# JuliaGaussianProcesses/AbstractGPs.jl

Hardware: AMD Instinct MI355X
Metric: logpdf+posterior throughput (points/sec, fp64) at N=65536; % MFMA roofline (higher is better)
Workload: dtype f64; 1 GPU; C4: GP(SqExponentialKernel()) on 65536 3-D points, sigma2=0.01, fp64, one (logpdf, posterior-fit) pair per step; n=65536, d=3, parallelism=1 GPU

## Files before the change

abstractgps.jl_amd/csrc/bulk_plan.hpp:

```cpp
#pragma once
#include <algorithm>
#include <cstddef>
#include <vector>

namespace gpmi {

static inline double lower_count(long M, long N, long row0, long col0) {
    const long a = row0 - col0 + 1;
    const long i1 = std::min(std::max(1 - a, 0L), M);
    const long i2 = std::max(i1, std::min(std::max(N - a, 0L), M));
    const double mid = (double)(i2 - i1) * (double)a + 0.5 * (double)(i1 + i2 - 1) * (double)(i2 - i1);
    return mid + (double)(M - i2) * (double)N;
}

static inline bool strassen_shape_rule(long min_rows, long M, long N, long K) {
    return min_rows > 0 && std::min(M, N) >= std::max(256L, min_rows) && M % 256 == 0 && N % 256 == 0 && K % 32 == 0;
}
static inline long strassen_split_rule(long min_rows, long m, long K) {
    const long h = (m / 2) / 256 * 256;
    return strassen_shape_rule(min_rows, h, h, K) ? h : 0;
}
static inline size_t strassen_ws_rule(long ldpad, long M, long N, long K) { return (size_t)5 * (size_t)(M / 2 + N / 2) * (size_t)(K / 2 + ldpad); }
static inline long plan_tiles(long M, long N, int lower) {
    const long tm = (M + 127) / 128, tn = (N + 127) / 128;
// ... 38 lines not shown
    size_t ws_elems = 0;
    std::vector<PlanLaunch> ungrouped;
    size_t nprobs() const { return list[0].size() + list[1].size() + list[2].size() + list[3].size(); }
};

namespace plan_detail {
struct Builder {
    BulkPlan& p;
    long min_rows, ldpad;
    std::vector<PlanProb> classical;

    void rect(long c_off, long a_off, long b_off, long M, long N) {
        if (M <= 0 || N <= 0) return;
        PlanProb e{};
        e.c_off = c_off; e.a_off = a_off; e.b_off = b_off;
        e.M = M; e.N = N; e.K = p.K;
        e.block = -1;
        classical.push_back(e);
        p.ungrouped.push_back(PlanLaunch{0, M, N, p.K, 1, 0});
    }
    void product(int launch, int product, int block, long c_off, long c2off, int s1, int s2, int a_src, long a_off, int b_src, long b_off, long mh, long nh, long kh) {
        PlanProb e{};
        e.c_off = c_off; e.a_off = a_off; e.b_off = b_off;
        e.a_src = a_src; e.b_src = b_src;
        e.M = mh; e.N = nh; e.K = kh;
        e.beta0 = 1; e.c2off = c2off; e.s1 = s1; e.s2 = s2;
        e.block = block; e.product = product;
        p.list[launch].push_back(e);
    }
    void strassen(long c_off, long a_off, long b_off, long M, long N) {
        const long K = p.K;
        if (!strassen_shape_rule(min_rows, M, N, K)) return rect(c_off, a_off, b_off, M, N);
        const long mh = M / 2, nh = N / 2, kh = K / 2, lds = p.lds, ldp = p.ldp;
        const long pa = mh * lds, pb = nh * lds;
        const int bi = (int)p.blocks.size();
        const long sa = (long)p.ws_elems, sb = sa + 5 * pa;
        p.blocks.push_back(PlanBlock{c_off, a_off, b_off, M, N, K, sa, 5 * (pa + pb)});
        p.ws_elems += (size_t)(5 * (pa + pb));
        p.sums.push_back(PlanSums{a_off, mh, kh, 0, sa, pa});
        p.sums.push_back(PlanSums{b_off, nh, kh, 1, sb, pb});
        const long dn = nh, dm = mh * p.ldc;
        product(0, 1, bi, c_off, dm + dn, 1, 1, 1, sa, 1, sb, mh, nh, kh);
        product(1, 2, bi, c_off + dm, dn, 1, -1, 1, sa + pa, 0, b_off, mh, nh, kh);
        product(1, 5, bi, c_off + dn, -dn, 1, -1, 1, sa + 2 * pa, 0, b_off + nh * ldp + kh, mh, nh, kh);
        product(2, 3, bi, c_off + dn, dm, 1, 1, 0, a_off, 1, sb + pb, mh, nh, kh);
        product(2, 4, bi, c_off, dm, 1, 1, 0, a_off + mh * ldp + kh, 1, sb + 2 * pb, mh, nh, kh);
        product(3, 6, bi, c_off + dm + dn, 0, 1, 0, 1, sa + 3 * pa, 1, sb + 3 * pb, mh, nh, kh);
        product(3, 7, bi, c_off, 0, 1, 0, 1, sa + 4 * pa, 1, sb + 4 * pb, mh, nh, kh);
        p.ungrouped.push_back(PlanLaunch{1, mh, kh, 0, 1, 0});
        p.ungrouped.push_back(PlanLaunch{1, nh, kh, 0, 1, 0});
        p.ungrouped.push_back(PlanLaunch{0, mh, nh, kh, 1, 0});
        for (int i = 0; i < 3; ++i) p.ungrouped.push_back(PlanLaunch{0, mh, nh, kh, 2, 0});
    }
    void syrk(long roff, long mrows, long m) {
        const long K = p.K, ldc = p.ldc, ldp = p.ldp;
        const long h = strassen_split_rule(min_rows, m, K);
        if (h == 0) {
            PlanProb e{};
            e.c_off = roff * ldc + roff; e.a_off = roff * ldp; e.b_off = roff * ldp;
            e.M = mrows; e.N = m; e.K = K;
            e.lower = 1; e.roff = roff;
            e.block = -1;
            classical.push_back(e);
            p.ungrouped.push_back(PlanLaunch{0, mrows, m, K, 1, 1});
            return;
        }
        const long b = m - h, bs = b / 256 * 256;
        syrk(roff, h, h);
        strassen((roff + h) * ldc + roff, (roff + h) * ldp, roff * ldp, bs, h);
        if (b > bs) rect((roff + h + bs) * ldc + roff, (roff + h + bs) * ldp, roff * ldp, b - bs, h);
        syrk(roff + h, b, b);
        if (mrows > m) rect((roff + m) * ldc + roff, (roff + m) * ldp, roff * ldp, mrows - m, m);
    }
};
}

static inline BulkPlan bulk_plan_build(long mrows, long m, long K, long row0, long ldc, long ldp, long min_rows, long ldpad) {
    BulkPlan p;
    p.mrows = mrows; p.m = m; p.K = K; p.row0 = row0; p.ldc = ldc; p.ldp = ldp;
    p.lds = K / 2 + ldpad;
    plan_detail::Builder bd{p, min_rows, ldpad, {}};
    bd.syrk(0, mrows, m);
    double work[4];
    for (int l = 0; l < 4; ++l) {
        work[l] = 0;
        for (auto& e : p.list[l]) work[l] += (double)plan_tiles(e.M, e.N, e.lower) * (double)e.K;
    }
    std::stable_sort(bd.classical.begin(), bd.classical.end(), [](const PlanProb& a, const PlanProb& b) {
        return plan_tiles(a.M, a.N, a.lower) * a.K > plan_tiles(b.M, b.N, b.lower) * b.K;
    });
    for (auto& e : bd.classical) {
        int l = 0;
        for (int i = 1; i < 4; ++i)
            if (work[i] < work[l]) l = i;
        work[l] += (double)plan_tiles(e.M, e.N, e.lower) * (double)e.K;
        p.list[l].push_back(e);
    }
    for (int l = 0; l < 4; ++l) {
        std::stable_sort(p.list[l].begin(), p.list[l].end(), [](const PlanProb& a, const PlanProb& b) {
            if (a.K != b.K) return a.K > b.K;
            return plan_tiles(a.M, a.N, a.lower) > plan_tiles(b.M, b.N, b.lower);
        });
        long t = 0;
        for (auto& e : p.list[l]) {
            e.tile0 = t;
            e.ntiles = plan_tiles(e.M, e.N, e.lower);
            t += e.ntiles;
            const double elems = e.lower ? lower_count(e.M, e.N, row0 + e.roff, row0 + e.roff) : (double)e.M * (double)e.N;
            p.flops[l] += 2.0 * (double)e.K * elems;
            p.bytes[l] += 16.0 * elems * (e.c2off ? 2 : 1) + 8.0 * (double)e.K * (double)(e.M + e.N);
        }
        p.ntiles[l] = t;
    }
    return p;
}

struct GrpProb {
    double* C;
    const double* A;
    const double* B;
    long ldc, lda, ldb;
    long row0, col0;
    long c2off;
    int M, N, K;
    int lower, tn, beta0, s1, s2;
    int tile0;
    int pad_[5];
};
static_assert(sizeof(GrpProb) == 128, "one table entry is 128 bytes");

static inline GrpProb plan_entry(const BulkPlan& p, const PlanProb& e, double* C, const double* P, const double* ws) {
    GrpProb q{};
    q.C = C + e.c_off;
    q.A = (e.a_src ? ws : P) + e.a_off;
    q.B = (e.b_src ? ws : P) + e.b_off;
    q.ldc = p.ldc;
    q.lda = e.a_src ? p.lds : p.ldp;
    q.ldb = e.b_src ? p.lds : p.ldp;
    q.row0 = q.col0 = e.lower ? p.row0 + e.roff : 0;
    q.c2off = e.c2off;
    q.M = (int)e.M; q.N = (int)e.N; q.K = (int)e.K;
    q.lower = e.lower;
    q.tn = (int)((e.N + 127) / 128);
    q.beta0 = e.beta0; q.s1 = e.s1; q.s2 = e.s2;
    q.tile0 = (int)e.tile0;
    return q;
}

}
```

abstractgps.jl_amd/csrc/engine.hpp:

```cpp
#pragma once
#include <hip/hip_runtime.h>
#include <stdint.h>

#include <array>
#include <atomic>
#include <memory>
#include <mutex>
#include <set>
#include <string>
#include <unordered_map>
#include <vector>

#include "../../include/gpmi355.h"
#include "bulk_plan.hpp"

namespace gpmi {
struct GridMap {
    int lower;
    int P, p, Q, q;
    long nb;
    long row0, col0;
    int compact;
    int tn, dt;
    int tm;
// ... 11 lines not shown
struct KSum {
    enum { MAXT = 8, MAXFT = 4, MAXF = 16, MAXTH = 64, MAXD = 16 };
    int nterms, nth;
    int t0[MAXT + 1];
    int tv[MAXT];
    int kind[MAXF];
    int ns[MAXF];
    int so[MAXF];
    int po[MAXF];
    double th[MAXTH];
};
static_assert(sizeof(KSum) < 1024, "the composite kernel descriptor travels as a kernel argument");
}

int32_t set_hip_err(hipError_t e, const char* what, int line);
int32_t set_arg_err(int i, const char* msg);
int32_t set_err_text(int32_t status, const std::string& msg);
#define HIPCHK(expr)                                                   \
    do {                                                               \
        hipError_t e_ = (expr);                                        \
        if (e_ != hipSuccess) return set_hip_err(e_, #expr, __LINE__); \
    } while (0)
#define RC(expr)                \
    do {                        \
        int32_t rc_ = (expr);   \
        if (rc_ != 0) return rc_; \
    } while (0)

static inline long round_up(long v, long m) { return (v + m - 1) / m * m; }
static const double LOG2PI = 1.8378770664093454835606594728112;

template <class F> static inline auto by_dtype(int dtype, F&& f) { return dtype == 0 ? f(double()) : f(float()); }
static inline void put(void* out, int dtype, size_t i, double v) {
    if (dtype == 0) ((double*)out)[i] = v;
    else ((float*)out)[i] = (float)v;
}

struct FreeBlock {
    void* p;
    size_t bytes;
};

struct gp_ctx {
    int device = 0;
    hipStream_t sm = nullptr;
    hipStream_t sp = nullptr;
    void* pin = nullptr;
    size_t pin_bytes = 0;
    hipStream_t sq = nullptr;
    bool own_sm = false;
    std::mutex mu;
    long nb = -1;
    long nb_small = 4096, nb_large = 2048;
    int lookahead = 1;
    long lookahead_min_n = 24576;
    int time_kernels = 0;
    int sched = 0;
    long trsv_nb = 256;
    long leaf_group = 128;
    int deterministic = 0;
    int leaf_v2 = 1;
    int leaf_xr = 0;
    int upd128 = 1;
    long updk_max_k = 512;
    long updk_tall_k = 256;
    long updk_tall_m = 8192;
    int updk_rt = 0;
    int leaf_cols = 128;
    int gemm_streamk = 1;
    int num_cus = 256;
    long sk_max_tiles = 4096;
    long sk_min_k = 0;
    int sk_scope = 0;
    long gemm_pad_lds = 0;
    long gemm_pad_f32 = 0;
    int gemm_pipe = 1;
    long dib_nb = 2048;
    bool gemm_pad_set = false;
    bool gemm_pad_user = false;
    long vfe_ks = 2048;
    int vfe_overlap = 1;
    int vfe_sk = 0;
    int vfe_dual = 0;
    long vfe_inv_nb = 512;
    long strassen_min_rows = 8192;
    long strassen_min_rows_large = 4096;
    bool strassen_min_rows_set = false;
    long strassen_v = 8192;
    int strassen_group = 1;
    long strassen_group_min_rows = 8192;
    void* plan_pin = nullptr;
    size_t plan_pin_bytes = 0;
    hipEvent_t plan_ev = nullptr;
    bool grp_pad_set = false;
    int xcd_swizzle = 0;
    long xcd_min_tiles = 256;
    long ldpad = 32;
    long dense_stage_mb = 64;
    gp_timings tm{};
    std::vector<FreeBlock> pool;
    std::unordered_map<void*, size_t> blk;
    size_t pool_bytes = 0;
    size_t pool_cap = (size_t)96 << 30;
    int alloc_poison = 0;
    int64_t batch_grad_problems = 0;
    int64_t batch_pgrad_problems = 0;
    int64_t batch_gradx_problems = 0;
    int64_t batch_joint_problems = 0;
    long vfe_chunk = 0;
    std::vector<hipEvent_t> ev_pool;
    size_t ev_used = 0;
    struct GemmRec {
        hipEvent_t a, b;
        double flops, bytes;
        long M, N, K;
        long nprob, ntiles;
        int stream;
    };
    std::vector<GemmRec> gemm_recs;
    hipEvent_t ev_phase[4] = {nullptr, nullptr, nullptr, nullptr};
    int* info_dev = nullptr;
    int* ticket_dev = nullptr;
    void* w_ws = nullptr;
    size_t w_ws_bytes = 0;
    double* scal_dev = nullptr;
    long scal_cap = 0;
    std::atomic<int> refs{1};
    bool dead = false;
    struct gp_multi* multi = nullptr;
};

struct SkScope {
    gp_ctx* c;
    explicit SkScope(gp_ctx* c_) : c(c_) { ++c->sk_scope; }
    ~SkScope() { --c->sk_scope; }
};


extern std::mutex g_reg_mu;
extern std::set<void*> g_live;
void reg_add(void* p);
bool reg_take(void* p);
bool reg_has(void* p);
// ... 175 lines not shown
```

abstractgps.jl_amd/csrc/gpmi355.hip:

```cpp
#include "kernels.hpp"

#include <algorithm>
#include <atomic>
#include <cmath>
#include <cstdio>
#include <cstdlib>
#include <cstring>
#include <mutex>
#include <set>
#include <memory>
#include <string>
#include <thread>
#include <type_traits>
#include <unordered_map>
#include <vector>

using namespace gpmi;

static thread_local std::string g_err;
int32_t set_err_text(int32_t status, const std::string& msg) {
    g_err = msg;
    return status;
}
int32_t set_hip_err(hipError_t e, const char* what, int line) {
// ... 318 lines not shown
        g.c2stride = c2s;
        g.s1 = s1;
        g.s2 = s2;
        g.nbatch = nb;
        g.cstride = cs;
        g.astride = as;
        g.bstride = bs;
        return launch_gemm<double>(c, s, c1, ldc, a, la, b, lb, mh, nh, kh, g);
    };
    const long dn = nh, dm = mh * ldc;
    RC(prod(1, C, 0, dm + dn, 0, 1, 1, SA, lds, 0, SB, lds, 0));
    RC(prod(2, C + dm, dn - dm, dn, -2 * dn, 1, -1, SA + pa, lds, pa, B, ldb, nh * ldb + kh));
    RC(prod(2, C + dn, -dn, dm, 0, 1, 1, A, lda, mh * lda + kh, SB + pb, lds, pb));
    RC(prod(2, C + dm + dn, -(dm + dn), 0, 0, 1, 0, SA + 3 * pa, lds, pa, SB + 3 * pb, lds, pb));
    return 0;
}

static int32_t syrk_lower_split(gp_ctx* c, hipStream_t s, const StrassenWs& ws, double* C, long ldc, const double* P, long ldp, long mrows, long m, long K,
                                long row0) {
    const long h = ws.p ? strassen_split(c, m, K) : 0;
    if (h == 0) return launch_gemm<double>(c, s, C, ldc, P, ldp, P, ldp, mrows, m, K, plain_map(1, row0, row0));
    const long b = m - h, bs = b / 256 * 256;
    RC(syrk_lower_split(c, s, ws, C, ldc, P, ldp, h, h, K, row0));
    RC(gemm_nt_strassen(c, s, ws, C + h * ldc, ldc, P + h * ldp, ldp, P, ldp, bs, h, K));
    if (b > bs) RC(launch_gemm<double>(c, s, C + (h + bs) * ldc, ldc, P + (h + bs) * ldp, ldp, P, ldp, b - bs, h, K, plain_map(0, 0, 0)));
    RC(syrk_lower_split(c, s, ws, C + h * ldc + h, ldc, P + h * ldp, ldp, b, b, K, row0 + h));
    if (mrows > m) RC(launch_gemm<double>(c, s, C + m * ldc, ldc, P + m * ldp, ldp, P, ldp, mrows - m, m, K, plain_map(0, 0, 0)));
    return 0;
}
static size_t syrk_split_ws_elems(const gp_ctx* c, long m, long K) {
    return strassen_split(c, m, K) ? strassen_ws_elems(c, m / 2 + 256, m / 2 + 256, K) : 0;
}

static bool group_applies(const gp_ctx* c, long m, long K, long ldp, const double* P) {
    return c->strassen_group && !c->xcd_swizzle && m >= c->strassen_group_min_rows && strassen_split(c, m, K) != 0 && ldp % 2 == 0 && ((uintptr_t)P & 15) == 0;
}
struct GroupedUpdate {
    BulkPlan plan;
    const double* P = nullptr;
    size_t tab0[4] = {0, 0, 0, 0};
};
struct PlanTables {
    std::vector<GroupedUpdate> upd;
    std::vector<GrpProb> host;
    size_t ws_elems = 0;
    GrpProb* dev = nullptr;
    void add(const gp_ctx* c, long mrows, long m, long K, long row0, long ldc, const double* P, long ldp) {
        GroupedUpdate u;
        u.plan = bulk_plan_build(mrows, m, K, row0, ldc, ldp, c->strassen_v, c->ldpad);
        u.P = P;
        ws_elems = std::max(ws_elems, u.plan.ws_elems);
        upd.push_back(std::move(u));
    }
    int32_t upload(gp_ctx* c, hipStream_t s, DevBufs& bufs, const std::vector<double*>& Cs, const double* ws) {
        for (size_t i = 0; i < upd.size(); ++i)
            for (int l = 0; l < 4; ++l) {
                upd[i].tab0[l] = host.size();
                for (const PlanProb& e : upd[i].plan.list[l]) host.push_back(plan_entry(upd[i].plan, e, Cs[i], upd[i].P, ws));
            }
        if (host.empty()) return 0;
        const size_t bytes = host.size() * sizeof(GrpProb);
        void* p = nullptr;
        RC(bufs.get(bytes, &p));
        dev = (GrpProb*)p;
        if (!c->plan_ev) HIPCHK(hipEventCreateWithFlags(&c->plan_ev, hipEventDisableTiming));
        HIPCHK(hipEventSynchronize(c->plan_ev));
        if (c->plan_pin_bytes < bytes) {
            if (c->plan_pin) (void)hipHostFree(c->plan_pin);
            c->plan_pin = nullptr;
            c->plan_pin_bytes = 0;
            HIPCHK(hipHostMalloc(&c->plan_pin, bytes + bytes / 4 + 4096, hipHostMallocDefault));
            c->plan_pin_bytes = bytes + bytes / 4 + 4096;
        }
        memcpy(c->plan_pin, host.data(), bytes);
        HIPCHK(hipMemcpyAsync(dev, c->plan_pin, bytes, hipMemcpyHostToDevice, s));
        HIPCHK(hipEventRecord(c->plan_ev, s));
        return 0;
    }
};

static int32_t launch_gemm_grp(gp_ctx* c, hipStream_t s, const GrpProb* tab, long nprob, long ntiles, double flops, double bytes, long K) {
    if (nprob <= 0 || ntiles <= 0) return 0;
    gp_ctx::GemmRec rec{};
    const bool timed = c->time_kernels != 0;
    if (timed) {
        RC(ctx_event(c, &rec.a, true));
        RC(ctx_event(c, &rec.b, true));
        rec.flops = flops;
        rec.bytes = bytes;
        rec.M = 0; rec.N = 0; rec.K = K;
        rec.nprob = nprob; rec.ntiles = ntiles;
        rec.stream = (s == c->sp);
        HIPCHK(hipEventRecord(rec.a, s));
    }
    const long pad = c->gemm_pad_user ? c->gemm_pad_lds : 0;
    if (pad > 0 && !c->grp_pad_set) {
        HIPCHK(hipFuncSetAttribute((const void*)gemm_nt_grp_kernel<double, 0>, hipFuncAttributeMaxDynamicSharedMemorySize, 32768));
        HIPCHK(hipFuncSetAttribute((const void*)gemm_nt_grp_kernel<double, 1>, hipFuncAttributeMaxDynamicSharedMemorySize, 32768));
        c->grp_pad_set = true;
    }
    if (c->gemm_pipe) hipLaunchKernelGGL((gemm_nt_grp_kernel<double, 1>), dim3((unsigned)ntiles), dim3(256), (size_t)pad, s, tab, (int)nprob);
    else hipLaunchKernelGGL((gemm_nt_grp_kernel<double, 0>), dim3((unsigned)ntiles), dim3(256), (size_t)pad, s, tab, (int)nprob);
    HIPCHK(hipGetLastError());
    if (timed) {
        HIPCHK(hipEventRecord(rec.b, s));
        c->gemm_recs.push_back(rec);
// ... 292 lines not shown
static int32_t trsm_back_cached(gp_ctx* c, hipStream_t s, T* X, long ldx, long M, long Mvalid, const T* A, long ld, long np, const DibCache& cache,
                                DevBufs& bufs, BackWs& ws) {
    if (M <= 0 || Mvalid <= 0) return 0;
    if (!cache.w || cache.nbi < 128 || c->dib_nb < 128) return trsv<T>(c, s, A, ld, np, X, ldx, (int)Mvalid, false);
    const long nbi = cache.nbi, ldw = cache.ldw;
    if (!ws.bt) {
        const size_t wb = sizeof(T) * (size_t)(np + 128) * ldw;
        void* S_probe = nullptr;
        if (bufs.get(wb, &ws.bt) != 0 || bufs.scratch(sizeof(T) * (size_t)(M + 128) * ldw, &S_probe) != 0) {
            ws.bt = nullptr;
            return trsv<T>(c, s, A, ld, np, X, ldx, (int)Mvalid, false);
        }
        HIPCHK(hipMemsetAsync(ws.bt, 0, wb, s));
    }
    void* S_v = nullptr;
    RC(bufs.scratch(sizeof(T) * (size_t)(M + 128) * ldw, &S_v));
    T* Bt = (T*)ws.bt;
    T* S = (T*)S_v;
    const T* W = (const T*)cache.w;
    std::vector<std::pair<long, long>> blocks;
    dib_ranges(0, np, nbi, blocks);
    for (long bi = (long)blocks.size() - 1; bi >= 0; --bi) {
        const long j0 = blocks[bi].first, n = blocks[bi].second;
        hipLaunchKernelGGL(transpose_rect_kernel<T>, dim3((unsigned)((n + 31) / 32), (unsigned)((n + 31) / 32)), dim3(256), 0, s, W + j0 * ldw, ldw, Bt, ldw, n, n, 1);
        HIPCHK(hipGetLastError());
        GridMap g = plain_map(0, 0, 0);
        g.beta0 = 1;
        RC(launch_gemm<T>(c, s, S, ldw, X + j0, ldx, Bt, ldw, M, n, n, g));
        HIPCHK(hipMemcpy2DAsync(X + j0, sizeof(T) * ldx, S, sizeof(T) * ldw, sizeof(T) * n, M, hipMemcpyDeviceToDevice, s));
        if (j0 > 0) {
            hipLaunchKernelGGL(transpose_rect_kernel<T>, dim3((unsigned)((j0 + 31) / 32), (unsigned)((n + 31) / 32)), dim3(256), 0, s, A + j0 * ld, ld, Bt, ldw, n, j0, 0);
            HIPCHK(hipGetLastError());
            RC(launch_gemm<T>(c, s, X, ldx, X + j0, ldx, Bt, ldw, M, j0, n, plain_map(0, 0, 0)));
        }
    }
    return 0;
}

template <typename T>
static int32_t potrf_full_la(gp_ctx* c, T* A, long lda, long np, long mtot, int* info_dev, long n_valid, double* logdet_dev, DevBufs* bufs);

template <typename T>
static int32_t potrf_full(gp_ctx* c, T* A, long lda, long np, long mtot, int* info_dev, long n_valid,
                          double* logdet_dev, DevBufs* bufs = nullptr) {
    if (c->nb == 0) return potrf_rec<T>(c, c->sm, A, lda, 0, np, mtot, info_dev, 0, n_valid, logdet_dev);
    return potrf_full_la<T>(c, A, lda, np, mtot, info_dev, n_valid, logdet_dev, bufs);
}

template <typename T>
static int32_t potrf_full_la(gp_ctx* c, T* A, long lda, long np, long mtot, int* info_dev, long n_valid,
                             double* logdet_dev, DevBufs* bufs) {
    long nb = c->nb;
    c->strassen_v = (!c->strassen_min_rows_set && np >= c->lookahead_min_n) ? c->strassen_min_rows_large : c->strassen_min_rows;
    if (nb < 0) nb = np < c->lookahead_min_n ? c->nb_small : c->nb_large;
    if (nb <= 0 || nb >= np) return potrf_rec<T>(c, c->sm, A, lda, 0, np, mtot, info_dev, 0, n_valid, logdet_dev);
    nb = round_up(nb, 128);
    const bool la = c->lookahead != 0 && np >= c->lookahead_min_n;
    hipStream_t sM = c->sm, sP = la ? c->sp : c->sm;
    hipEvent_t ev_u1 = nullptr, ev_panel = nullptr;
    StrassenWs ws;
    PlanTables tabs;
    std::vector<long> gidx;
    if constexpr (std::is_same<T, double>::value) {
        if (bufs) {
            size_t el = 0;
            std::vector<double*> Cs;
            for (long k = 0; k < np; k += nb) {
                const long nbk = std::min(nb, np - k), k1 = k + nbk;
                if (k1 >= np) break;
                const long k2 = k1 + std::min(nb, np - k1);
                long gi = -1;
                if (k2 < np) {
                    const double* P = A + k2 * lda + k;
                    if (group_applies(c, np - k2, nbk, lda, P)) {
                        gi = (long)tabs.upd.size();
                        tabs.add(c, mtot - k2, np - k2, nbk, k2, lda, P, lda);
                        Cs.push_back(A + k2 * lda + k2);
                    } else
                        el = std::max(el, syrk_split_ws_elems(c, np - k2, nbk));
                }
                gidx.push_back(gi);
            }
            el = std::max(el, tabs.ws_elems);
            if (el) {
                void* p = nullptr;
                RC(bufs->get(sizeof(double) * el, &p));
                ws.p = (double*)p;
                ws.elems = el;
            }
            RC(tabs.upload(c, c->sm, *bufs, Cs, ws.p));
        }
    }
    if (la) {
        RC(ctx_event(c, &ev_u1, false));
        HIPCHK(hipEventRecord(ev_u1, c->sm));
        HIPCHK(hipStreamWaitEvent(sP, ev_u1, 0));
    }
    for (long k = 0; k < np; k += nb) {
        const long nbk = std::min(nb, np - k);
        RC(potrf_rec<T>(c, sP, A, lda, k, nbk, mtot, info_dev, 0, n_valid, logdet_dev));
        const long k1 = k + nbk;
        if (la) {
            RC(ctx_event(c, &ev_panel, false));
            HIPCHK(hipEventRecord(ev_panel, sP));
            HIPCHK(hipStreamWaitEvent(sM, ev_panel, 0));
        }
        if (k1 >= np) break;
        const long nb1 = std::min(nb, np - k1);
        RC(launch_gemm<T>(c, sM, A + k1 * lda + k1, lda, A + k1 * lda + k, lda, A + k1 * lda + k, lda, mtot - k1, nb1, nbk, plain_map(1, k1, k1)));
        if (la) {
            RC(ctx_event(c, &ev_u1, false));
            HIPCHK(hipEventRecord(ev_u1, sM));
            HIPCHK(hipStreamWaitEvent(sP, ev_u1, 0));
        }
        const long k2 = k1 + nb1;
        if (k2 < np) {
            if constexpr (std::is_same<T, double>::value) {
                const size_t step = (size_t)(k / nb);
                if (step < gidx.size() && gidx[step] >= 0) RC(run_grouped(c, sM, tabs, (size_t)gidx[step], ws.p));
                else RC(syrk_lower_split(c, sM, ws, A + k2 * lda + k2, lda, A + k2 * lda + k, lda, mtot - k2, np - k2, nbk, k2));
            } else
                RC(launch_gemm<T>(c, sM, A + k2 * lda + k2, lda, A + k2 * lda + k, lda, A + k2 * lda + k, lda,
                                  mtot - k2, np - k2, nbk, plain_map(1, k2, k2)));
        }
    }
    return 0;
}

template <typename T>
static int32_t trsv(gp_ctx* c, hipStream_t s, const T* L, long ldl, long np, T* R, long ldr, int nrhs, bool fwd) {
    const int NBV = (int)c->trsv_nb;
    const bool k2 = NBV <= 256;
    const size_t smem = k2 ? sizeof(T) * (256 + 64 * 65 + 16 * 64 + 4 * 256) : sizeof(T) * (NBV + 64 * 65 + 16 * 64);
    const long nblk = (np + NBV - 1) / NBV;
    T* W = nullptr;
    RC(trtri_tiles<T>(c, s, L, ldl, np, &W));
    for (long bb = 0; bb < nblk; ++bb) {
        const long b = fwd ? bb : (nblk - 1 - bb);
        const long b0 = b * NBV;
        const int nbv = (int)std::min<long>(NBV, np - b0);
        if (fwd) {
            if (k2)
                hipLaunchKernelGGL((trsv_diag2_kernel<T, true>), dim3(1), dim3(1024), smem, s, L, ldl, b0, nbv, R, ldr, nrhs, (const T*)W);
            else
                hipLaunchKernelGGL((trsv_diag_kernel<T, true>), dim3(1), dim3(1024), smem, s, L, ldl, b0, nbv, R, ldr, nrhs, (const T*)W);
            HIPCHK(hipGetLastError());
            const long lo = b0 + nbv;
            if (lo < np) {
                hipLaunchKernelGGL(trsv_upd_fwd_kernel<T>, dim3((unsigned)((np - lo + 3) / 4)), dim3(256), 0, s, L,
                                   ldl, b0, nbv, lo, np, R, ldr, nrhs);
                HIPCHK(hipGetLastError());
            }
        } else {
            if (k2)
                hipLaunchKernelGGL((trsv_diag2_kernel<T, false>), dim3(1), dim3(1024), smem, s, L, ldl, b0, nbv, R, ldr, nrhs, (const T*)W);
            else
                hipLaunchKernelGGL((trsv_diag_kernel<T, false>), dim3(1), dim3(1024), smem, s, L, ldl, b0, nbv, R, ldr, nrhs, (const T*)W);
            HIPCHK(hipGetLastError());
            if (b0 > 0) {
                hipLaunchKernelGGL(trsv_upd_bwd_kernel<T>, dim3((unsigned)((b0 + 255) / 256), c->deterministic ? 1u : (unsigned)(nbv / 64)),
                                   dim3(256), 0, s, L, ldl, b0, nbv, R, ldr, nrhs);
                HIPCHK(hipGetLastError());
// ... 1103 lines not shown
        if (hipGetDeviceProperties(&prop, device) == hipSuccess && prop.multiProcessorCount > 0) c->num_cus = prop.multiProcessorCount;
    }
    int lo = 0, hi = 0;
    (void)hipDeviceGetStreamPriorityRange(&lo, &hi);
    hipError_t e = hipStreamCreateWithPriority(&c->sp, hipStreamNonBlocking, hi);
    if (e != hipSuccess) {
        if (c->own_sm) (void)hipStreamDestroy(c->sm);
        delete c;
        return set_hip_err(e, "hipStreamCreateWithPriority", __LINE__);
    }
    reg_add(c);
    *out = c;
    if (const char* s = getenv("GPMI_PARAMS")) {
        std::string all(s);
        size_t pos = 0;
        while (pos < all.size()) {
            size_t e = all.find(',', pos);
            if (e == std::string::npos) e = all.size();
            const std::string kv = all.substr(pos, e - pos);
            const size_t q = kv.find('=');
            if (q != std::string::npos) (void)gp_ctx_set_param(c, kv.substr(0, q).c_str(), atoll(kv.c_str() + q + 1));
            pos = e + 1;
        }
    }
    return 0;
}

int32_t gp_ctx_destroy(gp_ctx* c) {
    if (!c || !reg_take(c)) return set_arg_err(1, "not a live gp_ctx");
    gp_multi* multi = nullptr;
    {
        std::lock_guard<std::mutex> l(c->mu);
        (void)hipSetDevice(c->device);
        (void)hipStreamSynchronize(c->sm);
        (void)hipStreamSynchronize(c->sp);
        c->dead = true;
        multi = c->multi;
        c->multi = nullptr;
    }
    if (multi) multi_destroy(multi);
    (void)hipSetDevice(c->device);
    ctx_unref(c);
    return 0;
}

int32_t gp_ctx_set_param(gp_ctx* c, const char* name, int64_t v) {
    Guard gd(c);
    if (!gd.ok) return set_arg_err(1, "not a live gp_ctx");
    if (!name) return set_arg_err(2, "name is NULL");
    if (c->multi && multi_set_param(c, name, v) == 0) return 0;
    if (!strcmp(name, "nb")) c->nb = v < 0 ? -1 : (v == 0 ? 0 : round_up(v, 128));
    else if (!strcmp(name, "nb_small")) c->nb_small = (v <= 0) ? 0 : round_up(v, 128);
    else if (!strcmp(name, "nb_large")) c->nb_large = (v <= 0) ? 0 : round_up(v, 128);
    else if (!strcmp(name, "lookahead")) c->lookahead = v != 0;
    else if (!strcmp(name, "lookahead_min_n")) c->lookahead_min_n = std::max<int64_t>(0, v);
    else if (!strcmp(name, "time_kernels")) c->time_kernels = v != 0;
    else if (!strcmp(name, "xcd_swizzle")) c->xcd_swizzle = v != 0;
    else if (!strcmp(name, "strassen_min_rows")) {
        c->strassen_min_rows = v <= 0 ? 0 : round_up(v, 256);
        c->strassen_min_rows_set = true;
    } else if (!strcmp(name, "strassen_min_rows_large")) c->strassen_min_rows_large = v <= 0 ? 0 : round_up(v, 256);
    else if (!strcmp(name, "strassen_group")) c->strassen_group = v != 0;
    else if (!strcmp(name, "strassen_group_min_rows")) c->strassen_group_min_rows = std::max<int64_t>(256, round_up(v, 256));
    else if (!strcmp(name, "gemm_streamk")) c->gemm_streamk = v != 0;
    else if (!strcmp(name, "sk_max_tiles")) c->sk_max_tiles = v;
    else if (!strcmp(name, "sk_min_k")) c->sk_min_k = v;
    else if (!strcmp(name, "gemm_pipe")) c->gemm_pipe = v != 0;
    else if (!strcmp(name, "kmat_rows")) g_kmat_rows = v != 0;
    else if (!strcmp(name, "dib_nb")) c->dib_nb = v <= 0 ? 0 : std::min<int64_t>(round_up(std::max<int64_t>(v, 128), 128), 8192);
    else if (!strcmp(name, "gemm_pad_f32")) c->gemm_pad_f32 = std::min<int64_t>(std::max<int64_t>(0, v), 32768);
    else if (!strcmp(name, "gemm_pad_lds")) {
        c->gemm_pad_lds = std::min<int64_t>(std::max<int64_t>(0, v), 32768);
        c->gemm_pad_user = true;
    }
    else if (!strcmp(name, "trsv_nb")) c->trsv_nb = v >= 1024 ? 1024 : (v >= 512 ? 512 : (v >= 256 ? 256 : 128));
    else if (!strcmp(name, "deterministic")) c->deterministic = v != 0;
    else if (!strcmp(name, "leaf_v2")) c->leaf_v2 = v != 0;
    else if (!strcmp(name, "leaf_xr")) c->leaf_xr = v == 64 ? 64 : (v == 128 ? 128 : 0);
    else if (!strcmp(name, "leaf_cols")) c->leaf_cols = v == 64 ? 64 : 128;
    else if (!strcmp(name, "updk_max_k")) c->updk_max_k = std::max<int64_t>(0, v);
    else if (!strcmp(name, "updk_rt")) c->updk_rt = (int)v;
    else if (!strcmp(name, "updk_tall_k")) c->updk_tall_k = std::max<int64_t>(0, v);
    else if (!strcmp(name, "updk_tall_m")) c->updk_tall_m = std::max<int64_t>(0, v);
    else if (!strcmp(name, "upd128")) c->upd128 = v != 0;
    else if (!strcmp(name, "leaf_group")) c->leaf_group = v < 128 ? 64 : (v >= 512 ? 512 : (v >= 256 ? 256 : 128));
    else if (!strcmp(name, "xcd_min_tiles")) c->xcd_min_tiles = v;
    else if (!strcmp(name, "ldpad")) c->ldpad = round_up(std::max<int64_t>(0, v), 16);
    else if (!strcmp(name, "dense_stage_mb")) c->dense_stage_mb = std::min<int64_t>(std::max<int64_t>(1, v), 256);
    else if (!strcmp(name, "vfe_ks")) c->vfe_ks = std::max<int64_t>(512, round_up(v, 512));
    else if (!strcmp(name, "vfe_sk")) c->vfe_sk = v != 0;
    else if (!strcmp(name, "vfe_dual")) c->vfe_dual = v != 0;
    else if (!strcmp(name, "vfe_inv_nb")) c->vfe_inv_nb = v <= 0 ? 0 : round_up(v, 128);
    else if (!strcmp(name, "vfe_overlap")) c->vfe_overlap = v != 0;
    else if (!strcmp(name, "vfe_chunk")) c->vfe_chunk = v <= 0 ? 0 : std::max<int64_t>(2048, round_up(v, 2048));
    else if (!strcmp(name, "pool_cap_mb")) c->pool_cap = (size_t)std::max<int64_t>(0, v) << 20;
    else if (!strcmp(name, "alloc_poison")) c->alloc_poison = v != 0;
    else if (!strcmp(name, "lookahead_depth") || !strcmp(name, "dist_nb") || !strcmp(name, "copy_kernel") || !strcmp(name, "multi_debug_sync") ||
             !strcmp(name, "multi_check") || !strcmp(name, "multi_verify") || !strcmp(name, "multi_inject_fault") || !strcmp(name, "multi_dist_predict") || !strcmp(name, "multi_window") || !strcmp(name, "multi_timeout_s") || !strcmp(name, "multi_gemm_streamk") || !strcmp(name, "multi_leaf_cols")) return c->multi ? 0 : set_arg_err(2, "multi-device parameter on a single-device ctx");
    else return set_arg_err(2, "unknown parameter");
    return 0;
}

int32_t gp_ctx_get_param(gp_ctx* c, const char* name, int64_t* out) {
    Guard gd(c);
    if (!gd.ok) return set_arg_err(1, "not a live gp_ctx");
    if (!name) return set_arg_err(2, "name is NULL");
    if (!out) return set_arg_err(3, "out is NULL");
    if (c->multi && multi_get_param(c, name, out) == 0) return 0;
    if (!strcmp(name, "batch_grad_kernel_problems")) {
        *out = c->batch_grad_problems;
        return 0;
    }
    if (!strcmp(name, "batch_pgrad_kernel_problems")) {
        *out = c->batch_pgrad_problems;
        return 0;
    }
    if (!strcmp(name, "batch_gradx_kernel_problems")) {
        *out = c->batch_gradx_problems;
        return 0;
    }
    if (!strcmp(name, "batch_joint_kernel_problems")) {
        *out = c->batch_joint_problems;
        return 0;
    }
    const struct { const char* n; int64_t v; } tab[] = {
        {"nb", c->nb}, {"nb_small", c->nb_small}, {"nb_large", c->nb_large}, {"lookahead", c->lookahead}, {"lookahead_min_n", c->lookahead_min_n}, {"time_kernels", c->time_kernels},
        {"xcd_swizzle", c->xcd_swizzle}, {"strassen_min_rows", c->strassen_min_rows}, {"strassen_min_rows_large", c->strassen_min_rows_large}, {"strassen_group", c->strassen_group}, {"strassen_group_min_rows", c->strassen_group_min_rows}, {"xcd_min_tiles", c->xcd_min_tiles}, {"gemm_streamk", c->gemm_streamk},
        {"sk_max_tiles", c->sk_max_tiles}, {"sk_min_k", c->sk_min_k}, {"gemm_pipe", c->gemm_pipe}, {"gemm_pad_f32", c->gemm_pad_f32},
        {"gemm_pad_lds", c->gemm_pad_user ? c->gemm_pad_lds : 0}, {"trsv_nb", c->trsv_nb},  {"deterministic", c->deterministic},
        {"leaf_v2", c->leaf_v2}, {"leaf_xr", c->leaf_xr}, {"leaf_cols", c->leaf_cols}, {"updk_max_k", c->updk_max_k}, {"updk_rt", c->updk_rt},
        {"updk_tall_k", c->updk_tall_k}, {"updk_tall_m", c->updk_tall_m}, {"upd128", c->upd128}, {"leaf_group", c->leaf_group},
        {"ldpad", c->ldpad}, {"dense_stage_mb", c->dense_stage_mb}, {"vfe_ks", c->vfe_ks}, {"vfe_sk", c->vfe_sk}, {"vfe_dual", c->vfe_dual}, {"vfe_inv_nb", c->vfe_inv_nb}, {"vfe_overlap", c->vfe_overlap}, {"vfe_chunk", c->vfe_chunk},
        {"kmat_rows", g_kmat_rows.load()}, {"dib_nb", c->dib_nb}, {"pool_cap_mb", (int64_t)(c->pool_cap >> 20)}, {"alloc_poison", c->alloc_poison},
        {"pool_cached_mb", (int64_t)(c->pool_bytes >> 20)}, {"pool_blocks", (int64_t)c->pool.size()}};
    for (const auto& e : tab)
        if (!strcmp(name, e.n)) {
            *out = e.v;
            return 0;
        }
    return set_arg_err(2, "unknown parameter");
}

int32_t gp_ctx_trim(gp_ctx* c) {
    Guard gd(c);
    if (!gd.ok) return set_arg_err(1, "not a live gp_ctx");
    (void)hipSetDevice(c->device);
    (void)hipStreamSynchronize(c->sm);
    (void)hipStreamSynchronize(c->sp);
    while (!c->pool.empty()) pool_drop(c, c->pool.size() - 1);
    if (c->multi) multi_trim(c);
    return 0;
}

int32_t gp_get_timings(gp_ctx* c, gp_timings* out) {
    Guard gd(c);
    if (!gd.ok) return set_arg_err(1, "not a live gp_ctx");
    if (!out) return set_arg_err(2, "out is NULL");
    *out = c->tm;
    return 0;
}

extern "C++" int32_t pack_ksum(const gp_ksum* k, int d, int argi, KSum& ks, gp_kernel& kid) {
    if (!k) return set_arg_err(argi, "kernel is NULL");
    if (k->dtype != 0 && k->dtype != 1) return set_arg_err(argi, "dtype must be 0 (f64) or 1 (f32)");
    if (k->nterms < 1 || k->nterms > KSum::MAXT) return set_arg_err(argi, "composite kernel: 1..8 terms");
    if (!k->terms) return set_arg_err(argi, "composite kernel: terms is NULL");
    if (d > KSum::MAXD) return set_arg_err(argi, "composite kernel: D must be <= 16");
    ks = KSum{};
    int nf = 0, nth = 0;
    double vsum = 0;
    const char* too_many = "composite kernel: at most 64 entries in theta";
    for (int t = 0; t < k->nterms; ++t) {
        const gp_kterm& tm = k->terms[t];
        if (!(tm.variance > 0)) return set_arg_err(argi, "composite kernel: term variance must be > 0");
        if (tm.nfactors < 1 || tm.nfactors > KSum::MAXFT) return set_arg_err(argi, "composite kernel: 1..4 factors per term");
        if (!tm.factors) return set_arg_err(argi, "composite kernel: factors is NULL");
        if (nf + tm.nfactors > KSum::MAXF) return set_arg_err(argi, "composite kernel: at most 16 factors in all");
        if (nth >= KSum::MAXTH) return set_arg_err(argi, too_many);
        ks.t0[t] = nf;
// ... 1045 lines not shown
```

include/gpmi355.h:

```cpp
#ifndef GPMI355_H
#define GPMI355_H

#include <stdint.h>

#ifdef __cplusplus
extern "C" {
#endif

#define GPMI355_ABI_VERSION 4

typedef struct gp_ctx gp_ctx;
typedef struct gp_post gp_post;
typedef struct gp_vfe gp_vfe;

typedef struct {
    int32_t kind;
    int32_t dtype;
    double variance;
    int32_t nscale;
    const double* scale;
} gp_kernel;

typedef struct {
    int32_t kind;
    int32_t nscale;
    const double* scale;
    int32_t nparam;
    const double* param;
} gp_kfactor;
typedef struct {
    double variance;
    int32_t nfactors;
    const gp_kfactor* factors;
} gp_kterm;
typedef struct {
    int32_t dtype;
    int32_t nterms;
    const gp_kterm* terms;
} gp_ksum;

typedef struct {
    const void* data;
    int64_t n;
    int32_t d;
    int32_t layout;
} gp_points;

typedef struct {
    int32_t kind;
    double s;
    const void* diag;
} gp_noise;

typedef struct {
    double assemble_ms;
    double potrf_ms;
    double solve_ms;
    double total_ms;
    double gemm_ms;
    double gemm_flops;
    int64_t gemm_launches;
    double gemm_bytes;
} gp_timings;

int32_t gp_ctx_create(gp_ctx** out, int32_t device, void* stream_or_null);
int32_t gp_ctx_create_multi(gp_ctx** out, const int32_t* devices, int32_t ndev, int32_t P, int32_t Q, int32_t nb);
int32_t gp_ctx_multi_info(gp_ctx* ctx, int32_t* P, int32_t* Q, int32_t* nb, int32_t* comm, int32_t* depth);
int32_t gp_ctx_multi_stats(gp_ctx* ctx, int64_t* fits, int64_t* retries, int64_t* solves);
int32_t gp_multi_solve_trace(int32_t P, int32_t Q, int32_t nblk, const char* path);
int32_t gp_multi_solve_trace_ex(int32_t P, int32_t Q, int32_t nblk, int32_t flags, const char* path);
int32_t gp_multi_schedule_trace(int32_t P, int32_t Q, int32_t nblk, int32_t depth, int32_t comm, const char* path);
int32_t gp_ctx_destroy(gp_ctx* ctx);
#define GPMI355_PARAM_DEFAULTS                                                                                                   \
    "nb=-1,nb_small=4096,nb_large=2048,lookahead=1,lookahead_min_n=24576,time_kernels=0,xcd_swizzle=0,xcd_min_tiles=256,gemm_streamk=1,sk_max_tiles=4096," \
    "sk_min_k=0,gemm_pipe=1,gemm_pad_f32=0,gemm_pad_lds=0,trsv_nb=256,deterministic=0,leaf_v2=1,leaf_xr=0,leaf_cols=128,"    \
    "updk_max_k=512,updk_rt=0,updk_tall_k=256,updk_tall_m=8192,upd128=1,leaf_group=128,ldpad=32,vfe_ks=2048,vfe_sk=0,"          \
    "vfe_overlap=1,vfe_dual=0,vfe_inv_nb=512,vfe_chunk=0,kmat_rows=1,dib_nb=2048,pool_cap_mb=98304,dense_stage_mb=64,alloc_poison=0,strassen_min_rows=8192,strassen_min_rows_large=4096,strassen_group=1,strassen_group_min_rows=8192"
int32_t gp_ctx_set_param(gp_ctx* ctx, const char* name, int64_t value);
int32_t gp_ctx_get_param(gp_ctx* ctx, const char* name, int64_t* value_out);
int32_t gp_ctx_trim(gp_ctx* ctx);
int32_t gp_get_timings(gp_ctx* ctx, gp_timings* out);
const char* gp_last_error(void);
int32_t gp_abi_version(void);

int32_t gp_kernelmatrix(gp_ctx* ctx, const gp_kernel* k, const gp_points* x, const gp_points* y_or_null,
                        void* out);

int32_t gp_logpdf(gp_ctx* ctx, const gp_kernel* k, const gp_points* x, const gp_noise* noise,
                  const void* mean_or_null, const void* Y, int64_t ldy, int32_t ncols, void* out);

int32_t gp_logpdf_terms(gp_ctx* ctx, const gp_kernel* k, const gp_points* x, const gp_noise* noise, const void* mean_or_null,
                        const void* Y_or_null, int64_t ldy, int32_t ncols, void* logdet_out_or_null, void* sqmahal_out_or_null);

int32_t gp_posterior_fit(gp_ctx* ctx, const gp_kernel* k, const gp_points* x, const gp_noise* noise,
                         const void* mean_or_null, const void* y, gp_post** out, void* alpha_out_or_null,
                         void* logpdf_out_or_null);

int32_t gp_posterior_predict(gp_post* post, const gp_points* xs, const void* prior_mean_xs_or_null,
                             int32_t what, void* mean_out, void* var_out, void* cov_out);
int32_t gp_posterior_predict_grad(gp_post* post, const gp_points* xs, const void* prior_mean_xs_or_null, int32_t what,
                                  void* mean_out_or_null, void* var_out_or_null, void* dmean_out_or_null, void* dvar_out_or_null);
int32_t gp_posterior_logpdf(gp_post* post, const gp_points* xs, const void* prior_mean_xs_or_null, const gp_noise* noise,
                            const void* Y, int64_t ldy, int32_t ncols, void* out);
int32_t gp_posterior_rand(gp_post* post, const gp_points* xs, const void* prior_mean_xs_or_null, const gp_noise* noise,
                          const void* xi, int32_t ncols, void* out);

int32_t gp_logpdf_grad(gp_ctx* ctx, const gp_kernel* k, const gp_points* x, const gp_noise* noise, const void* mean_or_null,
                       const void* y, void* logpdf_out, double* dvariance_out, double* dscale_out, void* dnoise_out,
                       void* dy_out, void* dx_out);

int32_t gp_kernelmatrix_sum(gp_ctx* ctx, const gp_ksum* k, const gp_points* x, const gp_points* y_or_null, void* out);
int32_t gp_logpdf_sum(gp_ctx* ctx, const gp_ksum* k, const gp_points* x, const gp_noise* noise, const void* mean_or_null,
                      const void* Y, int64_t ldy, int32_t ncols, void* out);
int32_t gp_posterior_fit_sum(gp_ctx* ctx, const gp_ksum* k, const gp_points* x, const gp_noise* noise, const void* mean_or_null,
                             const void* y, gp_post** out, void* alpha_out_or_null, void* logpdf_out_or_null);
int32_t gp_logpdf_grad_sum(gp_ctx* ctx, const gp_ksum* k, const gp_points* x, const gp_noise* noise, const void* mean_or_null,
                           const void* y, void* logpdf_out, double* dtheta_out_or_null, void* dnoise_out_or_null,
                           void* dy_out_or_null);
int32_t gp_logpdf_grad_sum_x(gp_ctx* ctx, const gp_ksum* k, const gp_points* x, const gp_noise* noise, const void* mean_or_null,
                             const void* y, void* logpdf_out, double* dtheta_out_or_null, void* dnoise_out_or_null,
                             void* dy_out_or_null, void* dx_out_or_null);
int32_t gp_logpdf_terms_sum(gp_ctx* ctx, const gp_ksum* k, const gp_points* x, const gp_noise* noise, const void* mean_or_null,
                            const void* Y_or_null, int64_t ldy, int32_t ncols, void* logdet_out_or_null, void* sqmahal_out_or_null);

#define GPMI355_BATCH_MAX_N 768
int32_t gp_logpdf_batch(gp_ctx* ctx, int32_t nb, const gp_kernel* k, int32_t nx, const gp_points* x, const gp_noise* noise,
                        const void* const* mean_or_null, int32_t ny, const void* const* y, void* logpdf_out, int32_t* info_out,
// ... 144 lines not shown
```

Measured before the change: 49960 points/s.

## Apply Strassen grouped plan to lookahead panel update and enlarge block size for huge N

```diff
diff --git a/abstractgps.jl_amd/csrc/bulk_plan.hpp b/abstractgps.jl_amd/csrc/bulk_plan.hpp
--- a/abstractgps.jl_amd/csrc/bulk_plan.hpp
+++ b/abstractgps.jl_amd/csrc/bulk_plan.hpp
@@ -114,19 +114,19 @@
         p.ungrouped.push_back(PlanLaunch{0, mh, nh, kh, 1, 0});
         for (int i = 0; i < 3; ++i) p.ungrouped.push_back(PlanLaunch{0, mh, nh, kh, 2, 0});
     }
+    void leaf(long roff, long mrows, long m) {
+        PlanProb e{};
+        e.c_off = roff * p.ldc + roff; e.a_off = roff * p.ldp; e.b_off = roff * p.ldp;
+        e.M = mrows; e.N = m; e.K = p.K;
+        e.lower = 1; e.roff = roff;
+        e.block = -1;
+        classical.push_back(e);
+        p.ungrouped.push_back(PlanLaunch{0, mrows, m, p.K, 1, 1});
+    }
     void syrk(long roff, long mrows, long m) {
         const long K = p.K, ldc = p.ldc, ldp = p.ldp;
         const long h = strassen_split_rule(min_rows, m, K);
-        if (h == 0) {
-            PlanProb e{};
-            e.c_off = roff * ldc + roff; e.a_off = roff * ldp; e.b_off = roff * ldp;
-            e.M = mrows; e.N = m; e.K = K;
-            e.lower = 1; e.roff = roff;
-            e.block = -1;
-            classical.push_back(e);
-            p.ungrouped.push_back(PlanLaunch{0, mrows, m, K, 1, 1});
-            return;
-        }
+        if (h == 0) return leaf(roff, mrows, m);
         const long b = m - h, bs = b / 256 * 256;
         syrk(roff, h, h);
         strassen((roff + h) * ldc + roff, (roff + h) * ldp, roff * ldp, bs, h);
@@ -135,14 +135,7 @@
         if (mrows > m) rect((roff + m) * ldc + roff, (roff + m) * ldp, roff * ldp, mrows - m, m);
     }
 };
-}
-
-static inline BulkPlan bulk_plan_build(long mrows, long m, long K, long row0, long ldc, long ldp, long min_rows, long ldpad) {
-    BulkPlan p;
-    p.mrows = mrows; p.m = m; p.K = K; p.row0 = row0; p.ldc = ldc; p.ldp = ldp;
-    p.lds = K / 2 + ldpad;
-    plan_detail::Builder bd{p, min_rows, ldpad, {}};
-    bd.syrk(0, mrows, m);
+static inline void finish(BulkPlan& p, Builder& bd, long row0) {
     double work[4];
     for (int l = 0; l < 4; ++l) {
         work[l] = 0;
@@ -174,6 +167,34 @@
         }
         p.ntiles[l] = t;
     }
+}
+}
+
+static inline BulkPlan bulk_plan_build(long mrows, long m, long K, long row0, long ldc, long ldp, long min_rows, long ldpad) {
+    BulkPlan p;
+    p.mrows = mrows; p.m = m; p.K = K; p.row0 = row0; p.ldc = ldc; p.ldp = ldp;
+    p.lds = K / 2 + ldpad;
+    plan_detail::Builder bd{p, min_rows, ldpad, {}};
+    bd.syrk(0, mrows, m);
+    plan_detail::finish(p, bd, row0);
+    return p;
+}
+
+static inline long u1_block_rows(long u1_min_rows, long u1_min_k, long mrect, long nb1, long K) {
+    const long bs = mrect / 256 * 256;
+    return u1_min_rows > 0 && bs >= u1_min_rows && K >= u1_min_k && strassen_shape_rule(256, bs, nb1, K) ? bs : 0;
+}
+static inline BulkPlan u1_plan_build(long mrows, long mrect, long nb1, long K, long row0, long ldc, long ldp, long ldpad) {
+    BulkPlan p;
+    p.mrows = mrows; p.m = nb1; p.K = K; p.row0 = row0; p.ldc = ldc; p.ldp = ldp;
+    p.lds = K / 2 + ldpad;
+    plan_detail::Builder bd{p, 256, ldpad, {}};
+    const long bs = mrect / 256 * 256, carried = mrows - nb1 - mrect;
+    bd.leaf(0, nb1, nb1);
+    bd.strassen(nb1 * ldc, nb1 * ldp, 0, bs, nb1);
+    bd.rect((nb1 + bs) * ldc, (nb1 + bs) * ldp, 0, mrect - bs, nb1);
+    bd.rect((nb1 + mrect) * ldc, (nb1 + mrect) * ldp, 0, carried, nb1);
+    plan_detail::finish(p, bd, row0);
     return p;
 }
 
diff --git a/abstractgps.jl_amd/csrc/engine.hpp b/abstractgps.jl_amd/csrc/engine.hpp
--- a/abstractgps.jl_amd/csrc/engine.hpp
+++ b/abstractgps.jl_amd/csrc/engine.hpp
@@ -87,6 +87,7 @@
     std::mutex mu;
     long nb = -1;
     long nb_small = 4096, nb_large = 2048;
+    long nb_huge = 4096, nb_huge_min_n = 49152;
     int lookahead = 1;
     long lookahead_min_n = 24576;
     int time_kernels = 0;
@@ -124,6 +125,8 @@
     long strassen_v = 8192;
     int strassen_group = 1;
     long strassen_group_min_rows = 8192;
+    long strassen_u1_min_rows = 16384;
+    long strassen_u1_min_k = 4096;
     void* plan_pin = nullptr;
     size_t plan_pin_bytes = 0;
     hipEvent_t plan_ev = nullptr;
diff --git a/abstractgps.jl_amd/csrc/gpmi355.hip b/abstractgps.jl_amd/csrc/gpmi355.hip
--- a/abstractgps.jl_amd/csrc/gpmi355.hip
+++ b/abstractgps.jl_amd/csrc/gpmi355.hip
@@ -394,6 +394,13 @@
         ws_elems = std::max(ws_elems, u.plan.ws_elems);
         upd.push_back(std::move(u));
     }
+    void add_u1(const gp_ctx* c, long mrows, long mrect, long nb1, long K, long row0, long ldc, const double* P, long ldp) {
+        GroupedUpdate u;
+        u.plan = u1_plan_build(mrows, mrect, nb1, K, row0, ldc, ldp, c->ldpad);
+        u.P = P;
+        ws_elems = std::max(ws_elems, u.plan.ws_elems);
+        upd.push_back(std::move(u));
+    }
     int32_t upload(gp_ctx* c, hipStream_t s, DevBufs& bufs, const std::vector<double*>& Cs, const double* ws) {
         for (size_t i = 0; i < upd.size(); ++i)
             for (int l = 0; l < 4; ++l) {
@@ -792,7 +799,7 @@
                              double* logdet_dev, DevBufs* bufs) {
     long nb = c->nb;
     c->strassen_v = (!c->strassen_min_rows_set && np >= c->lookahead_min_n) ? c->strassen_min_rows_large : c->strassen_min_rows;
-    if (nb < 0) nb = np < c->lookahead_min_n ? c->nb_small : c->nb_large;
+    if (nb < 0) nb = (c->nb_huge_min_n > 0 && np >= c->nb_huge_min_n) ? c->nb_huge : np < c->lookahead_min_n ? c->nb_small : c->nb_large;
     if (nb <= 0 || nb >= np) return potrf_rec<T>(c, c->sm, A, lda, 0, np, mtot, info_dev, 0, n_valid, logdet_dev);
     nb = round_up(nb, 128);
     const bool la = c->lookahead != 0 && np >= c->lookahead_min_n;
@@ -801,6 +808,7 @@
     StrassenWs ws;
     PlanTables tabs;
     std::vector<long> gidx;
+    std::vector<long> uidx;
     if constexpr (std::is_same<T, double>::value) {
         if (bufs) {
             size_t el = 0;
@@ -809,8 +817,15 @@
                 const long nbk = std::min(nb, np - k), k1 = k + nbk;
                 if (k1 >= np) break;
                 const long k2 = k1 + std::min(nb, np - k1);
-                long gi = -1;
+                long gi = -1, ui = -1;
                 if (k2 < np) {
+                    const double* P1 = A + k1 * lda + k;
+                    if (c->strassen_v > 0 && !c->xcd_swizzle && lda % 2 == 0 && ((uintptr_t)P1 & 15) == 0 &&
+                        u1_block_rows(c->strassen_u1_min_rows, c->strassen_u1_min_k, np - k2, k2 - k1, nbk) > 0) {
+                        ui = (long)tabs.upd.size();
+                        tabs.add_u1(c, mtot - k1, np - k2, k2 - k1, nbk, k1, lda, P1, lda);
+                        Cs.push_back(A + k1 * lda + k1);
+                    }
                     const double* P = A + k2 * lda + k;
                     if (group_applies(c, np - k2, nbk, lda, P)) {
                         gi = (long)tabs.upd.size();
@@ -820,6 +835,7 @@
                         el = std::max(el, syrk_split_ws_elems(c, np - k2, nbk));
                 }
                 gidx.push_back(gi);
+                uidx.push_back(ui);
             }
             el = std::max(el, tabs.ws_elems);
             if (el) {
@@ -847,7 +863,16 @@
         }
         if (k1 >= np) break;
         const long nb1 = std::min(nb, np - k1);
-        RC(launch_gemm<T>(c, sM, A + k1 * lda + k1, lda, A + k1 * lda + k, lda, A + k1 * lda + k, lda, mtot - k1, nb1, nbk, plain_map(1, k1, k1)));
+        bool u1_grouped = false;
+        if constexpr (std::is_same<T, double>::value) {
+            const size_t step = (size_t)(k / nb);
+            if (step < uidx.size() && uidx[step] >= 0) {
+                RC(run_grouped(c, sM, tabs, (size_t)uidx[step], ws.p));
+                u1_grouped = true;
+            }
+        }
+        if (!u1_grouped)
+            RC(launch_gemm<T>(c, sM, A + k1 * lda + k1, lda, A + k1 * lda + k, lda, A + k1 * lda + k, lda, mtot - k1, nb1, nbk, plain_map(1, k1, k1)));
         if (la) {
             RC(ctx_event(c, &ev_u1, false));
             HIPCHK(hipEventRecord(ev_u1, sM));
@@ -2057,6 +2082,8 @@
     if (!strcmp(name, "nb")) c->nb = v < 0 ? -1 : (v == 0 ? 0 : round_up(v, 128));
     else if (!strcmp(name, "nb_small")) c->nb_small = (v <= 0) ? 0 : round_up(v, 128);
     else if (!strcmp(name, "nb_large")) c->nb_large = (v <= 0) ? 0 : round_up(v, 128);
+    else if (!strcmp(name, "nb_huge")) c->nb_huge = (v <= 0) ? 0 : round_up(v, 128);
+    else if (!strcmp(name, "nb_huge_min_n")) c->nb_huge_min_n = std::max<int64_t>(0, v);
     else if (!strcmp(name, "lookahead")) c->lookahead = v != 0;
     else if (!strcmp(name, "lookahead_min_n")) c->lookahead_min_n = std::max<int64_t>(0, v);
     else if (!strcmp(name, "time_kernels")) c->time_kernels = v != 0;
@@ -2065,6 +2092,8 @@
         c->strassen_min_rows = v <= 0 ? 0 : round_up(v, 256);
         c->strassen_min_rows_set = true;
     } else if (!strcmp(name, "strassen_min_rows_large")) c->strassen_min_rows_large = v <= 0 ? 0 : round_up(v, 256);
+    else if (!strcmp(name, "strassen_u1_min_rows")) c->strassen_u1_min_rows = v <= 0 ? 0 : round_up(v, 256);
+    else if (!strcmp(name, "strassen_u1_min_k")) c->strassen_u1_min_k = std::max<int64_t>(0, v);
     else if (!strcmp(name, "strassen_group")) c->strassen_group = v != 0;
     else if (!strcmp(name, "strassen_group_min_rows")) c->strassen_group_min_rows = std::max<int64_t>(256, round_up(v, 256));
     else if (!strcmp(name, "gemm_streamk")) c->gemm_streamk = v != 0;
@@ -2129,7 +2158,7 @@
         return 0;
     }
     const struct { const char* n; int64_t v; } tab[] = {
-        {"nb", c->nb}, {"nb_small", c->nb_small}, {"nb_large", c->nb_large}, {"lookahead", c->lookahead}, {"lookahead_min_n", c->lookahead_min_n}, {"time_kernels", c->time_kernels},
+        {"nb", c->nb}, {"nb_small", c->nb_small}, {"nb_large", c->nb_large}, {"nb_huge", c->nb_huge}, {"nb_huge_min_n", c->nb_huge_min_n}, {"strassen_u1_min_rows", c->strassen_u1_min_rows}, {"strassen_u1_min_k", c->strassen_u1_min_k}, {"lookahead", c->lookahead}, {"lookahead_min_n", c->lookahead_min_n}, {"time_kernels", c->time_kernels},
         {"xcd_swizzle", c->xcd_swizzle}, {"strassen_min_rows", c->strassen_min_rows}, {"strassen_min_rows_large", c->strassen_min_rows_large}, {"strassen_group", c->strassen_group}, {"strassen_group_min_rows", c->strassen_group_min_rows}, {"xcd_min_tiles", c->xcd_min_tiles}, {"gemm_streamk", c->gemm_streamk},
         {"sk_max_tiles", c->sk_max_tiles}, {"sk_min_k", c->sk_min_k}, {"gemm_pipe", c->gemm_pipe}, {"gemm_pad_f32", c->gemm_pad_f32},
         {"gemm_pad_lds", c->gemm_pad_user ? c->gemm_pad_lds : 0}, {"trsv_nb", c->trsv_nb},  {"deterministic", c->deterministic},
diff --git a/include/gpmi355.h b/include/gpmi355.h
--- a/include/gpmi355.h
+++ b/include/gpmi355.h
@@ -72,7 +72,7 @@
 int32_t gp_multi_schedule_trace(int32_t P, int32_t Q, int32_t nblk, int32_t depth, int32_t comm, const char* path);
 int32_t gp_ctx_destroy(gp_ctx* ctx);
 #define GPMI355_PARAM_DEFAULTS                                                                                                   \
-    "nb=-1,nb_small=4096,nb_large=2048,lookahead=1,lookahead_min_n=24576,time_kernels=0,xcd_swizzle=0,xcd_min_tiles=256,gemm_streamk=1,sk_max_tiles=4096," \
+    "nb=-1,nb_small=4096,nb_large=2048,nb_huge=4096,nb_huge_min_n=49152,strassen_u1_min_rows=16384,strassen_u1_min_k=4096,lookahead=1,lookahead_min_n=24576,time_kernels=0,xcd_swizzle=0,xcd_min_tiles=256,gemm_streamk=1,sk_max_tiles=4096," \
     "sk_min_k=0,gemm_pipe=1,gemm_pad_f32=0,gemm_pad_lds=0,trsv_nb=256,deterministic=0,leaf_v2=1,leaf_xr=0,leaf_cols=128,"    \
     "updk_max_k=512,updk_rt=0,updk_tall_k=256,updk_tall_m=8192,upd128=1,leaf_group=128,ldpad=32,vfe_ks=2048,vfe_sk=0,"          \
     "vfe_overlap=1,vfe_dual=0,vfe_inv_nb=512,vfe_chunk=0,kmat_rows=1,dib_nb=2048,pool_cap_mb=98304,dense_stage_mb=64,alloc_poison=0,strassen_min_rows=8192,strassen_min_rows_large=4096,strassen_group=1,strassen_group_min_rows=8192"
```

After: 51310 points/s (median of 6 runs). 1.03x the previous value.
